# oss0430/SRFRD

Hardware: NVIDIA B200
Metric: training seqs/sec; full-catalogue top-10 users/sec (higher is better)
Workload: dtype bf16

## Files before the change

include/srfrd_b200.h:

```cpp
#ifndef SRFRD_B200_H
#define SRFRD_B200_H

#include <stddef.h>
#include <stdint.h>

#ifdef __cplusplus
extern "C" {
#endif

#define SRFRD_ABI_VERSION 9
#if defined(__GNUC__)
#define SRFRD_API __attribute__((visibility("default")))
#else
#define SRFRD_API
#endif

SRFRD_API const char* srfrd_last_error(void);
SRFRD_API int srfrd_abi_version(void);
SRFRD_API int srfrd_device_check(void);

SRFRD_API int srfrd_embed_ln_fwd(const float* item_table, int64_t n_rows, int D, const float* pos_table,
                       const float* aux_table, int64_t n_aux, int F, int mode, const int64_t* seq,
                       const int64_t* aux_ids, int64_t B, int L, float item_scale, const float* ln_w,
                       const float* ln_b, float eps, void* x0_bf16, float* x0_f32, void* q_bf16, float* stats,
                       int ldx, float drop_p, uint64_t drop_seed, uint32_t drop_stream, const float* drop_step,
// ... 138 lines not shown
  int* last_row;
  int64_t cap;
} srfrd_pack_t;
SRFRD_API int srfrd_pack_plan(const int64_t* seq, const int64_t* keep, int64_t B, int L, const srfrd_pack_t* pk, void* stream);
SRFRD_API int srfrd_set_row_limit(const int* rows_dev);
SRFRD_API int srfrd_embed_ln_fwd_packed(const float* item_table, int64_t n_rows, int D, const float* pos_table,
                              const float* aux_table, int64_t n_aux, int F, int mode, const int64_t* seq,
                              const int64_t* aux_ids, int64_t B, int L, float item_scale, const float* ln_w,
                              const float* ln_b, float eps, void* x0_bf16, void* q_bf16, float* stats, int ldx,
                              float drop_p, uint64_t drop_seed, uint32_t drop_stream, const float* drop_step,
                              const int* row_tok, const int* rows_dev, int64_t cap_rows, void* stream);
SRFRD_API int srfrd_layernorm_fwd_rows(const void* x_bf16, int ldx, const float* w, const float* b, float eps, float* y_f32,
                             int ldy, const int* row_index, int64_t n, int H, void* stream);
SRFRD_API int srfrd_attention_packed_supported(int L, int H, int heads);
SRFRD_API int srfrd_attention_packed_oproj_supported(int L, int H, int heads);
SRFRD_API int srfrd_attention_fwd_packed(const void* q, int ldq, const void* k, const void* v, int ldkv, void* o, int ldo,
                               const srfrd_pack_t* pk, int L, int H, int heads, float drop_p, uint64_t seed,
                               uint32_t stream_id, const float* drop_step, void* stream, const void* wo, int ldw,
                               const float* bo, const void* res, int ldres, const float* ln_w, const float* ln_b,
                               float ln_eps, float* ln_stats, void* r, int ldr, void* y, int ldy);
SRFRD_API int srfrd_attention_bwd_packed(const void* dout, int lddo, const void* q, int ldq, const void* k, const void* v,
                               int ldkv, void* dq, int lddq, void* dk, void* dv, int lddkv, const srfrd_pack_t* pk,
                               int L, int H, int heads, float drop_p, uint64_t seed, uint32_t stream_id,
                               const float* drop_step, void* stream, const void* dr, int lddr, const void* woT, int ldw);
SRFRD_API int srfrd_score_loss_fused_packed(const float* h, int ldh, const float* item_table, const float* fake_table,
                                  const int64_t* pos, const int64_t* neg, const int64_t* prs, const int64_t* nrs,
                                  const float* w_pos, const float* w_neg, const float* norm, int D, int F,
                                  float* loss_acc, float* dh, int lddh, float* d_item, float* d_fake,
                                  const int* row_tok, const int* rows_dev, int64_t cap_rows, void* stream);
SRFRD_API int srfrd_embed_bwd_packed(const void* dx0_bf16, int ldx, const int64_t* seq, const int64_t* aux_ids,
                           const int* row_tok, const int* rows_dev, int64_t cap_rows, int L, int D, int F, int mode,
                           float item_scale, float* d_item, float* d_aux, float* d_pos, void* stream);

typedef struct {
  const float* bias1; const float* bias2;
// ... 38 lines not shown
```

srfrd_b200/_lib.py:

```python
from __future__ import annotations

import ctypes as C
import os

_HERE = os.path.dirname(os.path.abspath(__file__))
LIB_PATH = os.environ.get("SRFRD_B200_LIB") or os.path.join(_HERE, "lib", "libsrfrd_b200.so")

vp, i32, i64, f32, u32, u64 = C.c_void_p, C.c_int, C.c_int64, C.c_float, C.c_uint32, C.c_uint64


class GemmEpilogue(C.Structure):
    _fields_ = [("bias", vp), ("residual", vp), ("gate", vp), ("row_ids", vp), ("out_bf16", vp), ("out_f32", vp),
                ("ldr", i32), ("ldg", i32), ("ldc", i32), ("relu", i32), ("drop_p", f32), ("drop_stream", u32),
                ("drop_seed", u64), ("drop_step", vp),
                ("ln_out_bf16", vp), ("ln_w", vp), ("ln_b", vp), ("ln_stats", vp), ("ld_ln", i32), ("ln_eps", f32)]


class CastDesc(C.Structure):
    _fields_ = [("src", vp), ("src_ld", i32), ("dst", vp), ("dst_ld", i32), ("dst_t", vp), ("dst_t_ld", i32),
                ("rows", i32), ("cols", i32), ("dst_is_f32", i32)]


class Mlp2Epilogue(C.Structure):
    _fields_ = [("bias1", vp), ("bias2", vp), ("gate", vp), ("ldg", i32), ("relu1", i32), ("drop1_p", f32), ("drop2_p", f32),
# ... 51 lines not shown
    "srfrd_merge_topk_packed": [vp, i64, i32, i32, vp, vp, vp],
    "srfrd_catalogue_rank": [vp, i64, i64, i32, vp, i64, i64, i64, i32, i32, i32, vp, i32, vp, vp, vp, vp],
    "srfrd_attention_live_items": [vp, i64, i32, i32, vp, vp, vp, vp],
    "srfrd_set_attention_live": [vp, vp, vp, vp],
    "srfrd_merge_topk": [vp, vp, i64, i32, i32, vp, vp, vp],
    "srfrd_unpack_rows": [C.POINTER(RepackPart), i32, C.POINTER(PackDesc), i64, i32, vp],
    "srfrd_pack_rows": [C.POINTER(RepackPart), i32, C.POINTER(PackDesc), i64, i32, vp],
    "srfrd_dp_adam_step": [vp, vp, vp, i32, i32, i64, vp, vp, f32, f32, f32, f32, vp, vp, vp, vp, vp, i32, vp, vp],
    "srfrd_pack_plan": [vp, vp, i64, i32, C.POINTER(PackDesc), vp],
    "srfrd_set_row_limit": [vp],
    "srfrd_embed_ln_fwd_packed": [vp, i64, i32, vp, vp, i64, i32, i32, vp, vp, i64, i32, f32, vp, vp, f32, vp, vp, vp, i32,
                                  f32, u64, u32, vp, vp, vp, i64, vp],
    "srfrd_layernorm_fwd_rows": [vp, i32, vp, vp, f32, vp, i32, vp, i64, i32, vp],
    "srfrd_attention_packed_supported": [i32, i32, i32],
    "srfrd_attention_packed_oproj_supported": [i32, i32, i32],
    "srfrd_attention_fwd_packed": [vp, i32, vp, vp, i32, vp, i32, C.POINTER(PackDesc), i32, i32, i32, f32, u64, u32, vp, vp,
                                   vp, i32, vp, vp, i32, vp, vp, f32, vp, vp, i32, vp, i32],
    "srfrd_attention_bwd_packed": [vp, i32, vp, i32, vp, vp, i32, vp, i32, vp, vp, i32, C.POINTER(PackDesc), i32, i32, i32,
                                   f32, u64, u32, vp, vp, vp, i32, vp, i32],
    "srfrd_score_loss_fused_packed": [vp, i32, vp, vp, vp, vp, vp, vp, vp, vp, vp, i32, i32, vp, vp, i32, vp, vp, vp, vp,
                                      i64, vp],
    "srfrd_embed_bwd_packed": [vp, i32, vp, vp, vp, vp, i64, i32, i32, i32, i32, f32, vp, vp, vp, vp],
    "srfrd_sample_candidates": [vp, vp, vp, vp, i64, i32, i32, u64, vp, vp],
    "srfrd_candidate_rank": [vp, i32, vp, i64, i32, vp, i64, i32, vp, i32, vp, vp, i32, vp, vp, vp],
    "srfrd_add_user_term": [vp, i32, i64, i32, vp, i32, vp, vp, i32, vp],
    "srfrd_sample_batch": [vp, vp, vp, vp, vp, i32, i32, i32, i32, i32, u64, vp, vp, vp, vp, vp, vp, vp, vp, vp, vp],
}

_lib = None
_device_ok = False
launch_count = 0

# ... 1 lines not shown
def load() -> C.CDLL:
    global _lib
    if _lib is not None:
        return _lib
    if not os.path.exists(LIB_PATH):
        raise RuntimeError(
            f"srfrd_b200: {LIB_PATH} is not built. Run `make -C srfrd_b200/csrc` (needs nvcc, sm_100a). "
            "There is no CPU fallback.")
    lib = C.CDLL(LIB_PATH)
    lib.srfrd_last_error.restype = C.c_char_p
    lib.srfrd_last_error.argtypes = []
    for name, argtypes in SIGNATURES.items():
        fn = getattr(lib, name)
        fn.argtypes = argtypes
        fn.restype = C.c_int
    if lib.srfrd_abi_version() != 9:
        raise RuntimeError("srfrd_b200: ABI version mismatch between _lib.py and the built library")
    _lib = lib
    return lib


def require_device() -> None:
    global _device_ok
    if _device_ok:
        return
    lib = load()
    if lib.srfrd_device_check() != 0:
        raise RuntimeError("srfrd_b200: " + lib.srfrd_last_error().decode())
    _device_ok = True


# ... 24 lines not shown
```

srfrd_b200/csrc/attention_tc.cu:

```cuda
#include <stdlib.h>

#include "common.cuh"
#include "srfrd_b200.h"

namespace srfrd {

int attn_fwd_simt(const void* q, int ldq, const void* k, const void* v, int ldkv, void* o, int ldo, int64_t B, int L,
                  int H, int heads, float drop_p, uint64_t seed, uint32_t stream_id, const float* drop_step, void* stream);
int attn_bwd_simt(const void* dout, int lddo, const void* q, int ldq, const void* k, const void* v, int ldkv, void* dq,
                  int lddq, void* dk, void* dv, int lddkv, int64_t B, int L, int H, int heads, float drop_p,
                  uint64_t seed, uint32_t stream_id, const float* drop_step, void* stream);

bool attn_long_supported(int64_t B, int L, int H, int heads, int ldq, int ldkv);
int attn_long_fwd(const void* q, int ldq, const void* k, const void* v, int ldkv, void* o, int ldo, float* stats, int64_t B,
                  int L, int H, int heads, float drop_p, uint64_t seed, uint32_t stream_id, const float* drop_step,
                  void* stream);
int attn_long_bwd(const void* dout, int lddo, const void* q, int ldq, const void* k, const void* v, int ldkv, const void* o,
                  int ldo, float* stats, void* dq, int lddq, void* dk, void* dv, int lddkv, int64_t B, int L, int H, int heads,
                  float drop_p, uint64_t seed, uint32_t stream_id, const float* drop_step, void* stream);

static constexpr int TILE = 128;
static constexpr int OPB = TILE * 64 * 2;
static constexpr int ATC_THREADS = 192;

struct AttnTc {
  int64_t T;
  int L, hd, heads, spt, n_tiles, kblocks;
  int tma_o;
  int debug;
  float scale, scale_log2e;
  bf16* o; int ldo;
  bf16 *dq, *dk, *dv; int lddq, lddkv;
  uint64_t drop_seed; uint32_t drop_thresh, drop_stream; float drop_scale; const float* drop_step;
  const int* pk_rows;
  const int4* pk_info;
  const int* pk_tile_row0;
  const float *op_bias, *ln_w, *ln_b; float* ln_stats; float ln_eps;
  bf16 *op_r, *op_y; int ldr, ldy;
};

__device__ __forceinline__ uint32_t sw128(int r, int c) {
  return (uint32_t)(r * 128 + ((((c >> 3) ^ (r & 7)) << 4) | ((c & 7) << 1)));
}

struct RowInfo {
  int r; int64_t t; bool owned; int jlo, jhi, l; int64_t bh;
  float pm;
  int jbase;
};
__device__ __forceinline__ RowInfo row_info_pk(const AttnTc& p, int row0, int M, int h, int quarter, int lane) {
  RowInfo ri;
  ri.r = quarter * 32 + lane;
  ri.t = (int64_t)row0 + ri.r;
// ... 108 lines not shown
  return y;
}

__device__ __forceinline__ void store_staged_rows(bf16* dst, int ld, int64_t row0, int col0, const uint8_t* blocks, int hd,
                                                  int n_own, int tid256) {
  const int cpr = hd >> 3;
  for (int i = tid256; i < n_own * cpr; i += 256) {
    const int r = i / cpr, ch = i - r * cpr;
    const uint4 v = *reinterpret_cast<const uint4*>(blocks + (ch >> 3) * OPB + sw128(r, (ch & 7) * 8));
    *reinterpret_cast<uint4*>(dst + (row0 + r) * ld + col0 + ch * 8) = v;
  }
}

static constexpr int AF_THREADS = 320;

__device__ __forceinline__ void out_proj_epilogue(const AttnTc& p, uint8_t* Qs, uint8_t* Vs, float* xsum, float* xsq,
                                               const float* sop, uint32_t tacc, uint64_t* proj_full, uint64_t* w_full,
                                               uint32_t ph, int r, int part, int quarter, int row0, int n_own) {
  mbar_wait2(proj_full, ph, w_full, ph);
  tc_fence_after();
  float ln_sum = 0.f, ln_sq = 0.f;
#pragma unroll 1
  for (int c = part * 32; c < p.hd; c += 64) {
    uint32_t raw[32];
    tmem_ld32(tacc + c, raw);
    uint8_t* blk = Vs + (c >> 6) * OPB;
    uint4 ax[4];
#pragma unroll
    for (int j = 0; j < 4; ++j)
      if (c + 8 * j < p.hd) ax[j] = *reinterpret_cast<const uint4*>(blk + sw128(r, (c & 63) + 8 * j));
// ... 20 lines not shown
  for (int c = part * 32; c < p.hd; c += 64) {
#pragma unroll
    for (int j = 0; j < 4; ++j) {
      if (c + 8 * j >= p.hd) break;
      const uint32_t off = (c >> 6) * OPB + sw128(r, (c & 63) + 8 * j);
      *reinterpret_cast<uint4*>(Qs + off) =
          lnf_apply8(*reinterpret_cast<const uint4*>(Vs + off), rstd, nb, sop + TILE + c + 8 * j, sop + 2 * TILE + c + 8 * j);
    }
  }
  if (part == 0 && r < n_own && p.ln_stats) *reinterpret_cast<float2*>(p.ln_stats + 2 * (size_t)(row0 + r)) = make_float2(mean, rstd);
  named_bar_sync_a(9, 256);
  store_staged_rows(p.op_r, p.ldr, row0, 0, Vs, p.hd, n_own, threadIdx.x);
  store_staged_rows(p.op_y, p.ldy, row0, 0, Qs, p.hd, n_own, threadIdx.x);
}

template <bool DROP, bool PK, bool OP>
__global__ void __launch_bounds__(AF_THREADS, 2)
attn_fwd_tc_kernel(const __grid_constant__ CUtensorMap tmQ, const __grid_constant__ CUtensorMap tmK,
                   const __grid_constant__ CUtensorMap tmV, const __grid_constant__ CUtensorMap tmO,
                   const __grid_constant__ CUtensorMap tmW, const __grid_constant__ CUtensorMap tmR, AttnTc p) {
  extern __shared__ uint8_t smem_raw[];
  uint8_t* smem = reinterpret_cast<uint8_t*>((reinterpret_cast<uintptr_t>(smem_raw) + 1023) & ~uintptr_t(1023));
  const int opbytes = p.kblocks * OPB;
  uint8_t* Qs = smem;
  uint8_t* Ks = Qs + opbytes;
  uint8_t* Vs = Ks + max(p.kblocks, 2) * OPB;
  float* smax = reinterpret_cast<float*>(Vs + opbytes);
  float* ssum = smax + 2 * TILE;
  uint64_t* bars = reinterpret_cast<uint64_t*>(ssum + 2 * TILE);
  uint64_t *qk_full = bars, *v_full = bars + 1, *s_full = bars + 2, *p_full = bars + 3, *o_full = bars + 4,
           *kv_free = bars + 5, *q_free = bars + 6;
  uint64_t *w_full = bars + 7, *o_staged = bars + 8, *proj_full = bars + 9;
  uint32_t* tmem_slot = reinterpret_cast<uint32_t*>(bars + 10);
  float* sop = reinterpret_cast<float*>(bars + 16);
  const int warp = threadIdx.x >> 5, lane = threadIdx.x & 31;

  if (warp == 8 && lane == 0) {
    tma_prefetch_desc(&tmQ); tma_prefetch_desc(&tmK); tma_prefetch_desc(&tmV); tma_prefetch_desc(&tmO);
    if (OP) { tma_prefetch_desc(&tmW); tma_prefetch_desc(&tmR); }
    mbar_init(qk_full, 1); mbar_init(v_full, 1); mbar_init(s_full, 1); mbar_init(p_full, 8); mbar_init(o_full, 1);
    mbar_init(kv_free, 1); mbar_init(q_free, 1);
    mbar_init(w_full, 1); mbar_init(o_staged, 1); mbar_init(proj_full, 1);
    fence_barrier_init();
  }
  if (warp == 9) { tmem_alloc(tmem_slot, 256); tmem_relinquish(); }
  tc_fence_before();
  __syncthreads();
  tc_fence_after();
  const uint32_t tmem_base = *tmem_slot;
  const uint32_t tS = tmem_base, tO = tmem_base + 128;
  pdl_prologue_done();
  if (DROP) p.drop_seed = mix_seed(p.drop_seed, p.drop_step);
  const int pk_M = PK ? __ldg(p.pk_rows) : 0;
  const int n_items = (PK ? __ldg(p.pk_rows + 2) : p.n_tiles) * p.heads;

  if (warp == 8) {
    uint32_t ph = 0;
    for (int it = blockIdx.x; it < n_items; it += gridDim.x, ph ^= 1) {
      const int tile = it / p.heads, h = it % p.heads;
      const int row0 = PK ? __ldg(p.pk_tile_row0 + tile) : tile * p.spt * p.L, col0 = h * p.hd;
      mbar_wait(q_free, ph ^ 1);
      if (!OP) mbar_wait(kv_free, ph ^ 1);
      AT_STAMP(0, it / gridDim.x);
      if (elect_one()) {
        mbar_expect_tx(qk_full, 2 * opbytes);
        for (int kb = 0; kb < p.kblocks; ++kb) {
          tma_load_2d(Qs + kb * OPB, &tmQ, qk_full, col0 + kb * 64, row0, SRFRD_EVICT_FIRST);
          tma_load_2d(Ks + kb * OPB, &tmK, qk_full, col0 + kb * 64, row0, SRFRD_EVICT_FIRST);
        }
        mbar_expect_tx(v_full, opbytes);
        for (int kb = 0; kb < p.kblocks; ++kb)
          tma_load_2d(Vs + kb * OPB, &tmV, v_full, col0 + kb * 64, row0, SRFRD_EVICT_FIRST);
      }
      __syncwarp();
      if (OP) {
        mbar_wait(kv_free, ph);
        if (elect_one()) {
          mbar_expect_tx(w_full, p.kblocks * (p.hd * 128 + OPB));
          for (int kb = 0; kb < p.kblocks; ++kb) {
            tma_load_2d(Ks + kb * OPB, &tmW, w_full, kb * 64, 0, SRFRD_EVICT_LAST);
            tma_load_2d(Vs + kb * OPB, &tmR, w_full, kb * 64, row0, SRFRD_EVICT_FIRST);
          }
        }
        __syncwarp();
      }
    }
  } else if (warp == 9) {
    const uint32_t idS = umma_idesc_bf16(TILE, TILE, 0, 0);
    const uint32_t idO = umma_idesc_bf16(TILE, p.hd, 0, 1);
    const uint32_t idW = umma_idesc_bf16(TILE, p.hd, 0, 0);
    const uint64_t dQ = umma_smem_desc(smem_u32(Qs), 0, 1024), dK = umma_smem_desc(smem_u32(Ks), 0, 1024);
    const uint64_t dP = umma_smem_desc(smem_u32(Ks), 0, 1024), dV = umma_smem_desc(smem_u32(Vs), OPB, 1024);
    uint32_t ph = 0;
    for (int it = blockIdx.x; it < n_items; it += gridDim.x, ph ^= 1) {
      mbar_wait(qk_full, ph);
      tc_fence_after();
      AT_STAMP(1, it / gridDim.x);
      if (elect_one()) {
        for (int kb = 0; kb < p.kblocks; ++kb) {
          const int ksteps = min(4, (p.hd - kb * 64) / 16);
          for (int k = 0; k < ksteps; ++k)
            umma_bf16(tS, dQ + (uint64_t)(kb * (OPB >> 4) + 2 * k), dK + (uint64_t)(kb * (OPB >> 4) + 2 * k), idS, (kb | k) != 0);
        }
        umma_commit(s_full);
      }
      __syncwarp();
      AT_STAMP(2, it / gridDim.x);
      mbar_wait(p_full, ph);
      mbar_wait(v_full, ph);
      tc_fence_after();
      AT_STAMP(3, it / gridDim.x);
      if (elect_one()) {
#pragma unroll
        for (int ks = 0; ks < 8; ++ks)
          umma_bf16(tO, dP + (uint64_t)((ks >> 2) * (OPB >> 4) + (ks & 3) * 2), dV + (uint64_t)(ks * 128), idO, ks != 0);
        umma_commit(kv_free);
        umma_commit(o_full);
      }
      __syncwarp();
      AT_STAMP(4, it / gridDim.x);
      if (OP) {
        mbar_wait2(o_staged, ph, w_full, ph);
        tc_fence_after();
        if (elect_one()) {
// ... 6 lines not shown
        }
        __syncwarp();
      }
    }
  } else {
    const int quarter = warp & 3, part = warp >> 2;
    const uint32_t lane_off = (uint32_t)(quarter * 32) << 16;
    const int r_first = quarter * 32;
    const int c_lo = PK ? (max(0, r_first - p.L) >> 5) : min(((r_first / p.L) * p.L) >> 5, quarter), c_hi = quarter;
    if (OP)
      for (int i = threadIdx.x; i < TILE; i += 256) {
        sop[i] = (p.op_bias && i < p.hd) ? __ldg(p.op_bias + i) : 0.f;
        sop[TILE + i] = i < p.hd ? __ldg(p.ln_w + i) : 0.f;
        sop[2 * TILE + i] = i < p.hd ? __ldg(p.ln_b + i) : 0.f;
      }
    uint32_t ph = 0;
    for (int it = blockIdx.x; it < n_items; it += gridDim.x, ph ^= 1) {
      const int tile = it / p.heads, h = it % p.heads;
      const int pk_row0 = PK ? __ldg(p.pk_tile_row0 + tile) : 0;
      RowInfo ri = PK ? row_info_pk(p, pk_row0, pk_M, h, quarter, lane) : row_info(p, tile, h, quarter, lane);
      if (!ri.owned) { ri.jlo = 1 << 20; ri.jhi = ri.jlo; }
      const unsigned span = (unsigned)(ri.jhi - ri.jlo);
      mbar_wait(s_full, ph);
      tc_fence_after();
      if (warp == 0) AT_STAMP(5, it / gridDim.x);
      const int c0 = c_lo + part, c1 = c_lo + part + 2;
      const int lo0 = (c0 <= c_hi) ? ri.jlo - c0 * 32 : (1 << 20);
      const int lo1 = (c1 <= c_hi) ? ri.jlo - c1 * 32 : (1 << 20);
      uint32_t raw0[32], raw1[32];
      tmem_ld32(tS + lane_off + min(c0, c_hi) * 32, raw0);
      tmem_ld32(tS + lane_off + min(c1, c_hi) * 32, raw1);
      tmem_ld_wait();
      float m = -INFINITY;
#pragma unroll
// ... 558 lines not shown
                          tmDO, tmDQ, tmDK, tmDV, tmDV, p));
  SRFRD_LAUNCH_CHECK();
  return 0;
}

static int packed_supported(int L, int H, int heads, int ldq, int ldkv) {
  if (!tc_supported(L, H, heads, ldq, ldkv)) return 0;
  const int hd = H / heads;
  return (L + 1 <= TILE) && (heads == 1 || hd % 64 == 0);
}

extern "C" int srfrd_attention_packed_supported(int L, int H, int heads) {
  return packed_supported(L, H, heads, 8, 8) && !getenv("SRFRD_ATTN_SIMT");
}

static size_t fwd_smem(int kblocks, bool op) {
  return (size_t)(2 * kblocks + (kblocks > 2 ? kblocks : 2)) * OPB + 4 * TILE * sizeof(float) + 1024 + 256 +
         (op ? 3 * TILE * sizeof(float) : 0);
}
static size_t bwd_smem(int kblocks, int hd, bool op) {
  return op ? (size_t)(4 * kblocks + 4) * OPB + 4096 + (size_t)kblocks * hd * 128 + 1024
            : (size_t)(4 * kblocks + 4) * OPB + 6 * TILE * sizeof(float) + 1024 + 256;
}
static constexpr size_t FWD_SMEM_MAX = 113 * 1024;
static constexpr size_t BWD_SMEM_MAX = 227 * 1024;

static int oproj_supported(int L, int H, int heads) {
  if (!packed_supported(L, H, heads, 8, 8) || heads != 1 || H > 128) return 0;
  const int kblocks = (H + 63) / 64;
  return (fwd_smem(kblocks, true) <= FWD_SMEM_MAX ? 1 : 0) | (bwd_smem(kblocks, H, true) <= BWD_SMEM_MAX ? 2 : 0);
}

extern "C" int srfrd_attention_packed_oproj_supported(int L, int H, int heads) {
  return getenv("SRFRD_ATTN_SIMT") ? 0 : oproj_supported(L, H, heads);
}

extern "C" int srfrd_attention_fwd_packed(const void* q, int ldq, const void* k, const void* v, int ldkv, void* o, int ldo,
                                          const srfrd_pack_t* pk, int L, int H, int heads, float drop_p, uint64_t seed,
                                          uint32_t stream_id, const float* drop_step, void* stream, const void* wo, int ldw,
                                          const float* bo, const void* res, int ldres, const float* ln_w, const float* ln_b,
                                          float ln_eps, float* ln_stats, void* r, int ldr, void* y, int ldy) {
  SRFRD_REQUIRE(q && k && v && o && pk && pk->rows && pk->row_info && pk->tile_row0, "attention_fwd_packed: null pointer");
  SRFRD_REQUIRE(packed_supported(L, H, heads, ldq, ldkv) && ldo % 8 == 0 && ((uintptr_t)o & 15) == 0,
                "attention_fwd_packed: unsupported shape (L=%d H=%d heads=%d)", L, H, heads);
  const bool op = wo != nullptr;
  if (op) {
    SRFRD_REQUIRE(oproj_supported(L, H, heads) & 1, "attention_fwd_packed: no fused out-projection for H=%d heads=%d", H, heads);
    SRFRD_REQUIRE(res && ln_w && ln_b && r && y, "attention_fwd_packed: fused out-projection needs residual, LayerNorm, r and y");
    SRFRD_REQUIRE(ldw % 8 == 0 && ldw >= H && ldres % 8 == 0 && ldr % 8 == 0 && ldy % 8 == 0 &&
                      (((uintptr_t)res | (uintptr_t)r | (uintptr_t)y | (uintptr_t)wo) & 15) == 0,
                  "attention_fwd_packed: bad out-projection operands");
  }
  AttnTc p = {};
  if (int rc = fill(p, 1, L, H, heads, drop_p, seed, stream_id, drop_step)) return rc;
  p.T = pk->cap;
  p.o = (bf16*)o; p.ldo = ldo; p.tma_o = 1;
  p.pk_rows = pk->rows; p.pk_info = (const int4*)pk->row_info; p.pk_tile_row0 = pk->tile_row0;
  CUtensorMap tmQ, tmK, tmV, tmW, tmR;
  if (int rc = make_tmap_bf16_2d(&tmQ, q, p.T, H, ldq, TILE, 64)) return rc;
  if (int rc = make_tmap_bf16_2d(&tmK, k, p.T, H, ldkv, TILE, 64)) return rc;
  if (int rc = make_tmap_bf16_2d(&tmV, v, p.T, H, ldkv, TILE, 64)) return rc;
  tmW = tmQ; tmR = tmQ;
  if (op) {
    if (int rc = make_tmap_bf16_2d(&tmW, wo, H, H, ldw, H, 64)) return rc;
    if (int rc = make_tmap_bf16_2d(&tmR, res, p.T, H, ldres, TILE, 64)) return rc;
    p.op_bias = bo; p.ln_w = ln_w; p.ln_b = ln_b; p.ln_stats = ln_stats; p.ln_eps = ln_eps;
    p.op_r = (bf16*)r; p.op_y = (bf16*)y; p.ldr = ldr; p.ldy = ldy;
  }
  const size_t smem = fwd_smem(p.kblocks, op);
  static bool attr = false;
  if (!attr) {
    SRFRD_CUDA(cudaFuncSetAttribute(attn_fwd_tc_kernel<false, true, false>, cudaFuncAttributeMaxDynamicSharedMemorySize, FWD_SMEM_MAX));
    SRFRD_CUDA(cudaFuncSetAttribute(attn_fwd_tc_kernel<true, true, false>, cudaFuncAttributeMaxDynamicSharedMemorySize, FWD_SMEM_MAX));
    SRFRD_CUDA(cudaFuncSetAttribute(attn_fwd_tc_kernel<false, true, true>, cudaFuncAttributeMaxDynamicSharedMemorySize, FWD_SMEM_MAX));
    SRFRD_CUDA(cudaFuncSetAttribute(attn_fwd_tc_kernel<true, true, true>, cudaFuncAttributeMaxDynamicSharedMemorySize, FWD_SMEM_MAX));
    attr = true;
  }
  int64_t grid = (pk->cap / 64 + 1) * heads;
  if (grid > 2 * num_sms()) grid = 2 * num_sms();
  auto kern = p.drop_thresh ? (op ? attn_fwd_tc_kernel<true, true, true> : attn_fwd_tc_kernel<true, true, false>)
                            : (op ? attn_fwd_tc_kernel<false, true, true> : attn_fwd_tc_kernel<false, true, false>);
  SRFRD_CUDA(launch_pdl(kern, dim3((unsigned)grid), dim3(AF_THREADS), smem, (cudaStream_t)stream, tmQ, tmK, tmV, tmQ, tmW, tmR, p));
  SRFRD_LAUNCH_CHECK();
  return 0;
}

extern "C" int srfrd_attention_bwd_packed(const void* dout, int lddo, const void* q, int ldq, const void* k, const void* v,
                                          int ldkv, void* dq, int lddq, void* dk, void* dv, int lddkv, const srfrd_pack_t* pk,
                                          int L, int H, int heads, float drop_p, uint64_t seed, uint32_t stream_id,
                                          const float* drop_step, void* stream, const void* dr, int lddr, const void* woT,
                                          int ldw) {
  const bool op = dr != nullptr;
  SRFRD_REQUIRE((op ? (woT != nullptr) : (dout != nullptr)) && q && k && v && dq && dk && dv && pk && pk->rows &&
                    pk->row_info && pk->tile_row0,
                "attention_bwd_packed: null pointer");
  SRFRD_REQUIRE(packed_supported(L, H, heads, ldq, ldkv) && (op || lddo % 8 == 0) && lddq % 8 == 0 && lddkv % 8 == 0 &&
                    (((uintptr_t)dq | (uintptr_t)dk | (uintptr_t)dv) & 15) == 0,
// ... 38 lines not shown
```

srfrd_b200/engine.py:

```python
from __future__ import annotations

import math
import os
from contextlib import contextmanager, nullcontext
from dataclasses import dataclass
from typing import Dict, List, Optional, Tuple

import torch

from . import ops

bf16 = torch.bfloat16
LN_EPS = 1e-8

KINDS = ("SRFR", "SRFRN", "SRFU_B", "SRFU_F", "SRFU_R", "SASRec")


@dataclass
class ModelSpec:
    kind: str
    item_number: int
    max_len: int
    D: int
    F: int = 0
# ... 491 lines not shown
            need = {"SRFU_B": 3, "SRFU_F": L + 1, "SRFU_R": 11}[s.kind]
            if s.n_labels < need and int(aux_ids.max()) >= s.n_labels:
                raise IndexError(f"index out of range in self: {s.kind} user label {int(aux_ids.max())} needs "
                                 f"number_of_labels >= {need}, got {s.n_labels}")
        aux_table = P.view(s.aux_key) if s.aux_key else None
        plan.build(seq, None if keep is None else keep.contiguous())
        hyb = self._hybrid_ws(B * L) if self.packed_mode(B, L) == "hybrid" else None
        live = None
        if hyb is not None and os.environ.get("SRFRD_LIVE_TILES", "1") != "0":
            live = self._live_tiles(B, L)
            live.build(plan)
        x = [ws[f"x{i}"][:T] for i in range(nb + 1)]
        row_ids = plan.row_ids
        fuse_ln = Hp <= 128 and os.environ.get("SRFRD_FUSE_LN", "1") != "0"
        fuse_oproj = self._fuse_oproj(hyb, L, fuse_ln) & 1
        with ops.row_limit(plan.rows):
            ops.embed_ln_fwd_packed(P.view(s.item_key), P.view(s.pos_key), aux_table, s.mode, seq, aux_ids, s.item_scale,
                                    P.view("attention_layernorms.0.weight"), P.view("attention_layernorms.0.bias"), LN_EPS,
                                    x[0], ws["Q0"][:T], ws["st1_0"][:T], plan,
                                    drop_p=p_drop if s.kind == "SASRec" else 0.0, drop_seed=seed, drop_stream=1, drop_step=step)
            for i in range(nb):
                Q, q, kv, o, r, y, h1 = (ws[f"{n}{i}"][:T] for n in ("Q", "q", "kv", "o", "r", "y", "h1"))
                with self._branch():
                    ops.gemm_tn(x[i], self.sh[f"wkv{i}"], out_bf16=kv, bias=self.bias("bkv", i))
                if i > 0 and not fuse_ln:
                    ops.layernorm_fwd(x[i], P.view(f"attention_layernorms.{i}.weight"), P.view(f"attention_layernorms.{i}.bias"),
                                      LN_EPS, y_bf16=Q, stats=ws[f"st1_{i}"][:T], H=H)
                ops.gemm_tn(Q, self.sh[f"wq{i}"], out_bf16=q, bias=self.bias("bq", i))
                self._join()
                if fuse_oproj:
                    ops.attention_fwd_packed(q, kv[:, :Hp], kv[:, Hp:], o, plan, L, H, s.num_heads, p_drop, seed, 10 + 4 * i, step,
                                             wo=self.sh[f"wo{i}"], bias=self.bias("bo", i), residual=Q, r=r, y=y,
                                             ln_w=P.view(f"forward_layernorms.{i}.weight"),
                                             ln_b=P.view(f"forward_layernorms.{i}.bias"), ln_eps=LN_EPS,
                                             ln_stats=ws[f"st2_{i}"][:T])
                elif hyb is None:
                    ops.attention_fwd_packed(q, kv[:, :Hp], kv[:, Hp:], o, plan, L, H, s.num_heads, p_drop, seed, 10 + 4 * i, step)
                else:
                    qd, kvd, od = hyb[f"qd{i}"][:B * L], hyb[f"kvd{i}"][:B * L], hyb[f"od{i}"][:B * L]
                    ops.unpack_rows([(q, qd, Hp, 0), (kv, kvd, 2 * Hp, 0)], plan)
                    with (live.active() if live is not None else nullcontext()):
                        ops.attention_fwd(qd, kvd[:, :Hp], kvd[:, Hp:], od, B, L, H, s.num_heads, p_drop, seed, 10 + 4 * i, step,
                                          stats=ws.get(f"ast{i}"))
                    ops.pack_rows([(od, o, Hp, 0)], plan)
                if fuse_oproj:
                    pass
                elif fuse_ln:
                    ops.gemm_tn(o, self.sh[f"wo{i}"], out_bf16=r, bias=self.bias("bo", i), residual=Q, ln_out=y,
                                ln_w=P.view(f"forward_layernorms.{i}.weight"), ln_b=P.view(f"forward_layernorms.{i}.bias"),
                                ln_eps=LN_EPS, ln_stats=ws[f"st2_{i}"][:T])
# ... 140 lines not shown
```

srfrd_b200/ops.py:

```python
from __future__ import annotations

import ctypes as C
from typing import Optional

import torch

from . import _lib
from contextlib import contextmanager

from ._lib import CastDesc, GemmEpilogue, Mlp2Epilogue, PackDesc, RepackPart, call

bf16 = torch.bfloat16


def _p(t: Optional[torch.Tensor]):
    return None if t is None else t.data_ptr()


def _stream():
    return torch.cuda.current_stream().cuda_stream


def _chk(t: torch.Tensor, dtype, name: str):
    if not t.is_cuda:
# ... 346 lines not shown
         0 if aux_table is None else aux_table.shape[0], F, mode, _p(seq), _p(aux_ids), B, L, float(item_scale), _p(ln_w),
         _p(ln_b), float(eps), _p(x0_bf16), _p(q_bf16), _p(stats), x0_bf16.stride(0), float(drop_p), int(drop_seed),
         int(drop_stream), _p(drop_step), _p(plan.row_tok), _p(plan.rows), plan.cap, _stream())


def layernorm_fwd_rows(x, w, b, eps, y_f32, row_index, n, H):
    _lib.require_device()
    call("srfrd_layernorm_fwd_rows", _p(x), x.stride(0), _p(w), _p(b), float(eps), _p(y_f32), y_f32.stride(0), _p(row_index),
         n, H, _stream())


def attention_packed_oproj_supported(L: int, H: int, heads: int) -> int:
    return int(_lib.load().srfrd_attention_packed_oproj_supported(int(L), int(H), int(heads)))


def attention_fwd_packed(q, k, v, o, plan: PackedPlan, L, H, heads, drop_p=0.0, seed=0, stream_id=0, drop_step=None,
                         wo=None, bias=None, residual=None, r=None, y=None, ln_w=None, ln_b=None, ln_eps=0.0, ln_stats=None):
    _lib.require_device()
    st = lambda t: 0 if t is None else t.stride(0)
    call("srfrd_attention_fwd_packed", _p(q), q.stride(0), _p(k), _p(v), k.stride(0), _p(o), o.stride(0), C.byref(plan.desc),
         L, H, heads, float(drop_p), int(seed), int(stream_id), _p(drop_step), _stream(), _p(wo), st(wo), _p(bias),
         _p(residual), st(residual), _p(ln_w), _p(ln_b), float(ln_eps), _p(ln_stats), _p(r), st(r), _p(y), st(y))


def attention_bwd_packed(dout, q, k, v, dq, dk, dv, plan: PackedPlan, L, H, heads, drop_p=0.0, seed=0, stream_id=0,
                         drop_step=None, dr=None, woT=None):
    st = lambda t: 0 if t is None else t.stride(0)
    call("srfrd_attention_bwd_packed", _p(dout), st(dout), _p(q), q.stride(0), _p(k), _p(v), k.stride(0), _p(dq),
         dq.stride(0), _p(dk), _p(dv), dk.stride(0), C.byref(plan.desc), L, H, heads, float(drop_p), int(seed),
         int(stream_id), _p(drop_step), _stream(), _p(dr), st(dr), _p(woT), st(woT))


def score_loss_fused_packed(h, item_table, fake_table, pos, neg, prs, nrs, w_pos, w_neg, norm, loss_acc, dh, d_item, d_fake,
                            plan: PackedPlan):
    D = item_table.shape[1]
    F = 0 if fake_table is None else fake_table.shape[1]
    call("srfrd_score_loss_fused_packed", _p(h), h.stride(0), _p(item_table), _p(fake_table), _p(pos), _p(neg), _p(prs),
# ... 49 lines not shown
```

Before: 9.857 million.

## Fuse Q and KV input projections into packed attention forward kernel

Adds an in-projection variant of the packed tensor-core attention forward kernel. It loads the raw Q input, the KV input and the Wq/Wkv weights by TMA, computes the Q, K and V projections with UMMA into TMEM, adds the biases and stages the results in shared memory. It also writes them to global memory, because the backward pass still needs them. The engine uses this path, and skips the separate wkv and wq GEMM launches plus the branch/join, whenever the fused out-projection is already active and the shape fits in TMEM and shared memory. The aim is fewer launches and less global round-tripping of q/kv, at the cost of more shared memory, serialized weight loads inside the kernel, and possibly repeated projection work per head item.

After: 10.03 million, median of 6. 1.02x the previous value.

```diff
diff --git a/include/srfrd_b200.h b/include/srfrd_b200.h
--- a/include/srfrd_b200.h
+++ b/include/srfrd_b200.h
@@ -8,7 +8,7 @@
 extern "C" {
 #endif
 
-#define SRFRD_ABI_VERSION 9
+#define SRFRD_ABI_VERSION 10
 #if defined(__GNUC__)
 #define SRFRD_API __attribute__((visibility("default")))
 #else
@@ -177,11 +177,14 @@
                              int ldy, const int* row_index, int64_t n, int H, void* stream);
 SRFRD_API int srfrd_attention_packed_supported(int L, int H, int heads);
 SRFRD_API int srfrd_attention_packed_oproj_supported(int L, int H, int heads);
+SRFRD_API int srfrd_attention_packed_inproj_supported(int L, int H, int heads);
 SRFRD_API int srfrd_attention_fwd_packed(const void* q, int ldq, const void* k, const void* v, int ldkv, void* o, int ldo,
                                const srfrd_pack_t* pk, int L, int H, int heads, float drop_p, uint64_t seed,
                                uint32_t stream_id, const float* drop_step, void* stream, const void* wo, int ldw,
                                const float* bo, const void* res, int ldres, const float* ln_w, const float* ln_b,
-                               float ln_eps, float* ln_stats, void* r, int ldr, void* y, int ldy);
+                               float ln_eps, float* ln_stats, void* r, int ldr, void* y, int ldy, const void* q_in,
+                               int ldq_in, const void* kv_in, int ldkv_in, const void* wq, int ldwq, const void* wkv,
+                               int ldwkv, const float* bq, const float* bkv);
 SRFRD_API int srfrd_attention_bwd_packed(const void* dout, int lddo, const void* q, int ldq, const void* k, const void* v,
                                int ldkv, void* dq, int lddq, void* dk, void* dv, int lddkv, const srfrd_pack_t* pk,
                                int L, int H, int heads, float drop_p, uint64_t seed, uint32_t stream_id,
diff --git a/srfrd_b200/_lib.py b/srfrd_b200/_lib.py
--- a/srfrd_b200/_lib.py
+++ b/srfrd_b200/_lib.py
@@ -89,8 +89,10 @@
     "srfrd_layernorm_fwd_rows": [vp, i32, vp, vp, f32, vp, i32, vp, i64, i32, vp],
     "srfrd_attention_packed_supported": [i32, i32, i32],
     "srfrd_attention_packed_oproj_supported": [i32, i32, i32],
+    "srfrd_attention_packed_inproj_supported": [i32, i32, i32],
     "srfrd_attention_fwd_packed": [vp, i32, vp, vp, i32, vp, i32, C.POINTER(PackDesc), i32, i32, i32, f32, u64, u32, vp, vp,
-                                   vp, i32, vp, vp, i32, vp, vp, f32, vp, vp, i32, vp, i32],
+                                   vp, i32, vp, vp, i32, vp, vp, f32, vp, vp, i32, vp, i32, vp, i32, vp, i32, vp, i32, vp, i32,
+                                   vp, vp],
     "srfrd_attention_bwd_packed": [vp, i32, vp, i32, vp, vp, i32, vp, i32, vp, vp, i32, C.POINTER(PackDesc), i32, i32, i32,
                                    f32, u64, u32, vp, vp, vp, i32, vp, i32],
     "srfrd_score_loss_fused_packed": [vp, i32, vp, vp, vp, vp, vp, vp, vp, vp, vp, i32, i32, vp, vp, i32, vp, vp, vp, vp,
@@ -122,7 +124,7 @@
         fn = getattr(lib, name)
         fn.argtypes = argtypes
         fn.restype = C.c_int
-    if lib.srfrd_abi_version() != 9:
+    if lib.srfrd_abi_version() != 10:
         raise RuntimeError("srfrd_b200: ABI version mismatch between _lib.py and the built library")
     _lib = lib
     return lib
diff --git a/srfrd_b200/csrc/attention_tc.cu b/srfrd_b200/csrc/attention_tc.cu
--- a/srfrd_b200/csrc/attention_tc.cu
+++ b/srfrd_b200/csrc/attention_tc.cu
@@ -37,6 +37,8 @@
   const int* pk_tile_row0;
   const float *op_bias, *ln_w, *ln_b; float* ln_stats; float ln_eps;
   bf16 *op_r, *op_y; int ldr, ldy;
+  const float *ip_bq, *ip_bkv;
+  bf16 *ip_q, *ip_k, *ip_v; int ip_ldq, ip_ldkv;
 };
 
 __device__ __forceinline__ uint32_t sw128(int r, int c) {
@@ -175,6 +177,50 @@
 
 static constexpr int AF_THREADS = 320;
 
+__device__ __forceinline__ void umma_in_proj(uint32_t tacc, uint64_t da, uint64_t db, uint32_t idesc, int hd) {
+  for (int kb = 0; kb * 64 < hd; ++kb) {
+    const int ksteps = min(4, (hd - kb * 64) / 16);
+    for (int k = 0; k < ksteps; ++k)
+      umma_bf16(tacc, da + (uint64_t)(kb * (OPB >> 4) + 2 * k), db + (uint64_t)(kb * (OPB >> 4) + 2 * k), idesc, (kb | k) != 0);
+  }
+}
+
+__device__ __forceinline__ void in_proj_epilogue(const AttnTc& p, uint8_t* Qs, uint8_t* Ks, uint8_t* Vs, const float* sip,
+                                              uint32_t tacc, uint64_t* qkv_full, uint64_t* qkv_staged, uint32_t ph, int r,
+                                              int part, int warp, int lane, int row0, int n_own) {
+  mbar_wait(qkv_full, ph);
+  tc_fence_after();
+  const bool own = r < n_own;
+#pragma unroll 1
+  for (int m = 0; m < 3; ++m) {
+    uint8_t* dst = m == 0 ? Qs : (m == 1 ? Ks : Vs);
+    bf16* gdst = m == 0 ? p.ip_q + (size_t)(row0 + r) * p.ip_ldq
+                        : (m == 1 ? p.ip_k : p.ip_v) + (size_t)(row0 + r) * p.ip_ldkv;
+    const float* bias = sip + m * TILE;
+#pragma unroll 1
+    for (int c = part * 32; c < p.hd; c += 64) {
+      uint32_t ro[32];
+      tmem_ld32(tacc + m * p.hd + c, ro);
+      tmem_ld_wait();
+      uint8_t* blk = dst + (c >> 6) * OPB;
+#pragma unroll
+      for (int u = 0; u < 4; ++u) {
+        if (c + 8 * u >= p.hd) break;
+        float v[8];
+#pragma unroll
+        for (int j = 0; j < 8; ++j) v[j] = __uint_as_float(ro[8 * u + j]) + bias[c + 8 * u + j];
+        const uint4 pk = make_uint4(pack_bf16x2(v[0], v[1]), pack_bf16x2(v[2], v[3]), pack_bf16x2(v[4], v[5]), pack_bf16x2(v[6], v[7]));
+        *reinterpret_cast<uint4*>(blk + sw128(r, (c & 63) + 8 * u)) = pk;
+        if (own) *reinterpret_cast<uint4*>(gdst + c + 8 * u) = pk;
+      }
+    }
+  }
+  tc_fence_before();
+  fence_proxy_async();
+  named_bar_sync_a(9, 256);
+  if (warp == 0 && lane == 0) mbar_arrive(qkv_staged);
+}
+
 __device__ __forceinline__ void out_proj_epilogue(const AttnTc& p, uint8_t* Qs, uint8_t* Vs, float* xsum, float* xsq,
                                                const float* sop, uint32_t tacc, uint64_t* proj_full, uint64_t* w_full,
                                                uint32_t ph, int r, int part, int quarter, int row0, int n_own) {
@@ -225,11 +271,12 @@
   store_staged_rows(p.op_y, p.ldy, row0, 0, Qs, p.hd, n_own, threadIdx.x);
 }
 
-template <bool DROP, bool PK, bool OP>
+template <bool DROP, bool PK, bool OP, bool IP = false>
 __global__ void __launch_bounds__(AF_THREADS, 2)
 attn_fwd_tc_kernel(const __grid_constant__ CUtensorMap tmQ, const __grid_constant__ CUtensorMap tmK,
                    const __grid_constant__ CUtensorMap tmV, const __grid_constant__ CUtensorMap tmO,
                    const __grid_constant__ CUtensorMap tmW, const __grid_constant__ CUtensorMap tmR, AttnTc p) {
+  static_assert(!IP || (PK && OP), "the fused in-projection runs on the packed, out-projection form only");
   extern __shared__ uint8_t smem_raw[];
   uint8_t* smem = reinterpret_cast<uint8_t*>((reinterpret_cast<uintptr_t>(smem_raw) + 1023) & ~uintptr_t(1023));
   const int opbytes = p.kblocks * OPB;
@@ -244,6 +291,9 @@
   uint64_t *w_full = bars + 7, *o_staged = bars + 8, *proj_full = bars + 9;
   uint32_t* tmem_slot = reinterpret_cast<uint32_t*>(bars + 10);
   float* sop = reinterpret_cast<float*>(bars + 16);
+  float* sip = sop + 3 * TILE;
+  uint64_t* ipbars = reinterpret_cast<uint64_t*>(sip + 3 * TILE);
+  uint64_t *q_done = ipbars, *ipw_full = ipbars + 1, *qkv_full = ipbars + 2, *qkv_staged = ipbars + 3;
   const int warp = threadIdx.x >> 5, lane = threadIdx.x & 31;
 
   if (warp == 8 && lane == 0) {
@@ -252,6 +302,7 @@
     mbar_init(qk_full, 1); mbar_init(v_full, 1); mbar_init(s_full, 1); mbar_init(p_full, 8); mbar_init(o_full, 1);
     mbar_init(kv_free, 1); mbar_init(q_free, 1);
     mbar_init(w_full, 1); mbar_init(o_staged, 1); mbar_init(proj_full, 1);
+    if (IP) { mbar_init(q_done, 1); mbar_init(ipw_full, 1); mbar_init(qkv_full, 1); mbar_init(qkv_staged, 1); }
     fence_barrier_init();
   }
   if (warp == 9) { tmem_alloc(tmem_slot, 256); tmem_relinquish(); }
@@ -273,7 +324,26 @@
       mbar_wait(q_free, ph ^ 1);
       if (!OP) mbar_wait(kv_free, ph ^ 1);
       AT_STAMP(0, it / gridDim.x);
-      if (elect_one()) {
+      if (IP) {
+        const int wbytes = p.hd * 128;
+        if (elect_one()) {
+          mbar_expect_tx(qk_full, 2 * opbytes + p.kblocks * wbytes);
+          for (int kb = 0; kb < p.kblocks; ++kb) {
+            tma_load_2d(Qs + kb * OPB, &tmQ, qk_full, kb * 64, row0, SRFRD_EVICT_FIRST);
+            tma_load_2d(Ks + kb * OPB, &tmK, qk_full, kb * 64, row0, SRFRD_EVICT_FIRST);
+            tma_load_2d(Vs + kb * OPB, &tmO, qk_full, kb * 64, 0, SRFRD_EVICT_LAST);
+          }
+        }
+        __syncwarp();
+        mbar_wait(q_done, ph);
+        if (elect_one()) {
+          mbar_expect_tx(ipw_full, 2 * p.kblocks * wbytes);
+          for (int kb = 0; kb < p.kblocks; ++kb) {
+            tma_load_2d(Vs + kb * OPB, &tmV, ipw_full, kb * 64, 0, SRFRD_EVICT_LAST);
+            tma_load_2d(Qs + kb * OPB, &tmV, ipw_full, kb * 64, p.hd, SRFRD_EVICT_LAST);
+          }
+        }
+      } else if (elect_one()) {
         mbar_expect_tx(qk_full, 2 * opbytes);
         for (int kb = 0; kb < p.kblocks; ++kb) {
           tma_load_2d(Qs + kb * OPB, &tmQ, qk_full, col0 + kb * 64, row0, SRFRD_EVICT_FIRST);
@@ -304,7 +374,27 @@
     const uint64_t dP = umma_smem_desc(smem_u32(Ks), 0, 1024), dV = umma_smem_desc(smem_u32(Vs), OPB, 1024);
     uint32_t ph = 0;
     for (int it = blockIdx.x; it < n_items; it += gridDim.x, ph ^= 1) {
-      mbar_wait(qk_full, ph);
+      if (IP) {
+        const uint64_t dVk = umma_smem_desc(smem_u32(Vs), 0, 1024);
+        mbar_wait(qk_full, ph);
+        tc_fence_after();
+        if (elect_one()) {
+          umma_in_proj(tmem_base, dQ, dVk, idW, p.hd);
+          umma_commit(q_done);
+        }
+        __syncwarp();
+        mbar_wait(ipw_full, ph);
+        tc_fence_after();
+        if (elect_one()) {
+          umma_in_proj(tmem_base + p.hd, dK, dVk, idW, p.hd);
+          umma_in_proj(tmem_base + 2 * p.hd, dK, dQ, idW, p.hd);
+          umma_commit(qkv_full);
+        }
+        __syncwarp();
+        mbar_wait(qkv_staged, ph);
+      } else {
+        mbar_wait(qk_full, ph);
+      }
       tc_fence_after();
       AT_STAMP(1, it / gridDim.x);
       if (elect_one()) {
@@ -318,7 +408,7 @@
       __syncwarp();
       AT_STAMP(2, it / gridDim.x);
       mbar_wait(p_full, ph);
-      mbar_wait(v_full, ph);
+      if (!IP) mbar_wait(v_full, ph);
       tc_fence_after();
       AT_STAMP(3, it / gridDim.x);
       if (elect_one()) {
@@ -355,10 +445,21 @@
         sop[TILE + i] = i < p.hd ? __ldg(p.ln_w + i) : 0.f;
         sop[2 * TILE + i] = i < p.hd ? __ldg(p.ln_b + i) : 0.f;
       }
+    if (IP) {
+      for (int i = threadIdx.x; i < TILE; i += 256) {
+        sip[i] = (p.ip_bq && i < p.hd) ? __ldg(p.ip_bq + i) : 0.f;
+        sip[TILE + i] = (p.ip_bkv && i < p.hd) ? __ldg(p.ip_bkv + i) : 0.f;
+        sip[2 * TILE + i] = (p.ip_bkv && i < p.hd) ? __ldg(p.ip_bkv + p.hd + i) : 0.f;
+      }
+      named_bar_sync_a(9, 256);
+    }
     uint32_t ph = 0;
     for (int it = blockIdx.x; it < n_items; it += gridDim.x, ph ^= 1) {
       const int tile = it / p.heads, h = it % p.heads;
       const int pk_row0 = PK ? __ldg(p.pk_tile_row0 + tile) : 0;
+      if (IP)
+        in_proj_epilogue(p, Qs, Ks, Vs, sip, tmem_base + lane_off, qkv_full, qkv_staged, ph, quarter * 32 + lane, part, warp,
+                         lane, pk_row0, __ldg(p.pk_tile_row0 + tile + 1) - pk_row0);
       RowInfo ri = PK ? row_info_pk(p, pk_row0, pk_M, h, quarter, lane) : row_info(p, tile, h, quarter, lane);
       if (!ri.owned) { ri.jlo = 1 << 20; ri.jhi = ri.jlo; }
       const unsigned span = (unsigned)(ri.jhi - ri.jlo);
@@ -947,9 +1048,9 @@
   return packed_supported(L, H, heads, 8, 8) && !getenv("SRFRD_ATTN_SIMT");
 }
 
-static size_t fwd_smem(int kblocks, bool op) {
+static size_t fwd_smem(int kblocks, bool op, bool ip = false) {
   return (size_t)(2 * kblocks + (kblocks > 2 ? kblocks : 2)) * OPB + 4 * TILE * sizeof(float) + 1024 + 256 +
-         (op ? 3 * TILE * sizeof(float) : 0);
+         (op ? 3 * TILE * sizeof(float) : 0) + (ip ? 3 * TILE * sizeof(float) + 64 : 0);
 }
 static size_t bwd_smem(int kblocks, int hd, bool op) {
   return op ? (size_t)(4 * kblocks + 4) * OPB + 4096 + (size_t)kblocks * hd * 128 + 1024
@@ -968,15 +1069,34 @@
   return getenv("SRFRD_ATTN_SIMT") ? 0 : oproj_supported(L, H, heads);
 }
 
+static bool inproj_supported(int L, int H, int heads) {
+  return (oproj_supported(L, H, heads) & 1) && 3 * H <= 256 && fwd_smem((H + 63) / 64, true, true) <= FWD_SMEM_MAX;
+}
+
+extern "C" int srfrd_attention_packed_inproj_supported(int L, int H, int heads) {
+  return !getenv("SRFRD_ATTN_SIMT") && inproj_supported(L, H, heads);
+}
+
 extern "C" int srfrd_attention_fwd_packed(const void* q, int ldq, const void* k, const void* v, int ldkv, void* o, int ldo,
                                           const srfrd_pack_t* pk, int L, int H, int heads, float drop_p, uint64_t seed,
                                           uint32_t stream_id, const float* drop_step, void* stream, const void* wo, int ldw,
                                           const float* bo, const void* res, int ldres, const float* ln_w, const float* ln_b,
-                                          float ln_eps, float* ln_stats, void* r, int ldr, void* y, int ldy) {
+                                          float ln_eps, float* ln_stats, void* r, int ldr, void* y, int ldy,
+                                          const void* q_in, int ldq_in, const void* kv_in, int ldkv_in, const void* wq,
+                                          int ldwq, const void* wkv, int ldwkv, const float* bq, const float* bkv) {
   SRFRD_REQUIRE(q && k && v && o && pk && pk->rows && pk->row_info && pk->tile_row0, "attention_fwd_packed: null pointer");
   SRFRD_REQUIRE(packed_supported(L, H, heads, ldq, ldkv) && ldo % 8 == 0 && ((uintptr_t)o & 15) == 0,
                 "attention_fwd_packed: unsupported shape (L=%d H=%d heads=%d)", L, H, heads);
-  const bool op = wo != nullptr;
+  const bool op = wo != nullptr, ip = wq != nullptr;
+  if (ip) {
+    SRFRD_REQUIRE(op && inproj_supported(L, H, heads), "attention_fwd_packed: no fused in-projection for H=%d heads=%d%s", H,
+                  heads, op ? "" : " without the fused out-projection");
+    SRFRD_REQUIRE(q_in && kv_in && wkv, "attention_fwd_packed: fused in-projection needs q_in, kv_in and wkv");
+    SRFRD_REQUIRE(ldq_in % 8 == 0 && ldkv_in % 8 == 0 && ldwq % 8 == 0 && ldwq >= H && ldwkv % 8 == 0 && ldwkv >= H &&
+                      (((uintptr_t)q_in | (uintptr_t)kv_in | (uintptr_t)wq | (uintptr_t)wkv | (uintptr_t)q | (uintptr_t)k |
+                        (uintptr_t)v) & 15) == 0,
+                  "attention_fwd_packed: bad in-projection operands");
+  }
   if (op) {
     SRFRD_REQUIRE(oproj_supported(L, H, heads) & 1, "attention_fwd_packed: no fused out-projection for H=%d heads=%d", H, heads);
     SRFRD_REQUIRE(res && ln_w && ln_b && r && y, "attention_fwd_packed: fused out-projection needs residual, LayerNorm, r and y");
@@ -989,10 +1109,20 @@
   p.T = pk->cap;
   p.o = (bf16*)o; p.ldo = ldo; p.tma_o = 1;
   p.pk_rows = pk->rows; p.pk_info = (const int4*)pk->row_info; p.pk_tile_row0 = pk->tile_row0;
-  CUtensorMap tmQ, tmK, tmV, tmW, tmR;
-  if (int rc = make_tmap_bf16_2d(&tmQ, q, p.T, H, ldq, TILE, 64)) return rc;
-  if (int rc = make_tmap_bf16_2d(&tmK, k, p.T, H, ldkv, TILE, 64)) return rc;
-  if (int rc = make_tmap_bf16_2d(&tmV, v, p.T, H, ldkv, TILE, 64)) return rc;
+  CUtensorMap tmQ, tmK, tmV, tmW, tmR, tmWq;
+  if (ip) {
+    if (int rc = make_tmap_bf16_2d(&tmQ, q_in, p.T, H, ldq_in, TILE, 64)) return rc;
+    if (int rc = make_tmap_bf16_2d(&tmK, kv_in, p.T, H, ldkv_in, TILE, 64)) return rc;
+    if (int rc = make_tmap_bf16_2d(&tmV, wkv, 2 * H, H, ldwkv, H, 64)) return rc;
+    if (int rc = make_tmap_bf16_2d(&tmWq, wq, H, H, ldwq, H, 64)) return rc;
+    p.ip_bq = bq; p.ip_bkv = bkv;
+    p.ip_q = (bf16*)q; p.ip_k = (bf16*)k; p.ip_v = (bf16*)v; p.ip_ldq = ldq; p.ip_ldkv = ldkv;
+  } else {
+    if (int rc = make_tmap_bf16_2d(&tmQ, q, p.T, H, ldq, TILE, 64)) return rc;
+    if (int rc = make_tmap_bf16_2d(&tmK, k, p.T, H, ldkv, TILE, 64)) return rc;
+    if (int rc = make_tmap_bf16_2d(&tmV, v, p.T, H, ldkv, TILE, 64)) return rc;
+    tmWq = tmQ;
+  }
   tmW = tmQ; tmR = tmQ;
   if (op) {
     if (int rc = make_tmap_bf16_2d(&tmW, wo, H, H, ldw, H, 64)) return rc;
@@ -1000,20 +1130,24 @@
     p.op_bias = bo; p.ln_w = ln_w; p.ln_b = ln_b; p.ln_stats = ln_stats; p.ln_eps = ln_eps;
     p.op_r = (bf16*)r; p.op_y = (bf16*)y; p.ldr = ldr; p.ldy = ldy;
   }
-  const size_t smem = fwd_smem(p.kblocks, op);
+  const size_t smem = fwd_smem(p.kblocks, op, ip);
   static bool attr = false;
   if (!attr) {
     SRFRD_CUDA(cudaFuncSetAttribute(attn_fwd_tc_kernel<false, true, false>, cudaFuncAttributeMaxDynamicSharedMemorySize, FWD_SMEM_MAX));
     SRFRD_CUDA(cudaFuncSetAttribute(attn_fwd_tc_kernel<true, true, false>, cudaFuncAttributeMaxDynamicSharedMemorySize, FWD_SMEM_MAX));
     SRFRD_CUDA(cudaFuncSetAttribute(attn_fwd_tc_kernel<false, true, true>, cudaFuncAttributeMaxDynamicSharedMemorySize, FWD_SMEM_MAX));
     SRFRD_CUDA(cudaFuncSetAttribute(attn_fwd_tc_kernel<true, true, true>, cudaFuncAttributeMaxDynamicSharedMemorySize, FWD_SMEM_MAX));
+    SRFRD_CUDA(cudaFuncSetAttribute(attn_fwd_tc_kernel<false, true, true, true>, cudaFuncAttributeMaxDynamicSharedMemorySize, FWD_SMEM_MAX));
+    SRFRD_CUDA(cudaFuncSetAttribute(attn_fwd_tc_kernel<true, true, true, true>, cudaFuncAttributeMaxDynamicSharedMemorySize, FWD_SMEM_MAX));
     attr = true;
   }
   int64_t grid = (pk->cap / 64 + 1) * heads;
   if (grid > 2 * num_sms()) grid = 2 * num_sms();
-  auto kern = p.drop_thresh ? (op ? attn_fwd_tc_kernel<true, true, true> : attn_fwd_tc_kernel<true, true, false>)
-                            : (op ? attn_fwd_tc_kernel<false, true, true> : attn_fwd_tc_kernel<false, true, false>);
-  SRFRD_CUDA(launch_pdl(kern, dim3((unsigned)grid), dim3(AF_THREADS), smem, (cudaStream_t)stream, tmQ, tmK, tmV, tmQ, tmW, tmR, p));
+  auto kern = p.drop_thresh ? (ip ? attn_fwd_tc_kernel<true, true, true, true>
+                                  : op ? attn_fwd_tc_kernel<true, true, true> : attn_fwd_tc_kernel<true, true, false>)
+                            : (ip ? attn_fwd_tc_kernel<false, true, true, true>
+                                  : op ? attn_fwd_tc_kernel<false, true, true> : attn_fwd_tc_kernel<false, true, false>);
+  SRFRD_CUDA(launch_pdl(kern, dim3((unsigned)grid), dim3(AF_THREADS), smem, (cudaStream_t)stream, tmQ, tmK, tmV, tmWq, tmW, tmR, p));
   SRFRD_LAUNCH_CHECK();
   return 0;
 }
diff --git a/srfrd_b200/engine.py b/srfrd_b200/engine.py
--- a/srfrd_b200/engine.py
+++ b/srfrd_b200/engine.py
@@ -529,6 +529,7 @@
         row_ids = plan.row_ids
         fuse_ln = Hp <= 128 and os.environ.get("SRFRD_FUSE_LN", "1") != "0"
         fuse_oproj = self._fuse_oproj(hyb, L, fuse_ln) & 1
+        fuse_inproj = fuse_oproj and ops.attention_packed_inproj_supported(L, H, s.num_heads)
         with ops.row_limit(plan.rows):
             ops.embed_ln_fwd_packed(P.view(s.item_key), P.view(s.pos_key), aux_table, s.mode, seq, aux_ids, s.item_scale,
                                     P.view("attention_layernorms.0.weight"), P.view("attention_layernorms.0.bias"), LN_EPS,
@@ -536,19 +537,22 @@
                                     drop_p=p_drop if s.kind == "SASRec" else 0.0, drop_seed=seed, drop_stream=1, drop_step=step)
             for i in range(nb):
                 Q, q, kv, o, r, y, h1 = (ws[f"{n}{i}"][:T] for n in ("Q", "q", "kv", "o", "r", "y", "h1"))
-                with self._branch():
-                    ops.gemm_tn(x[i], self.sh[f"wkv{i}"], out_bf16=kv, bias=self.bias("bkv", i))
-                if i > 0 and not fuse_ln:
-                    ops.layernorm_fwd(x[i], P.view(f"attention_layernorms.{i}.weight"), P.view(f"attention_layernorms.{i}.bias"),
-                                      LN_EPS, y_bf16=Q, stats=ws[f"st1_{i}"][:T], H=H)
-                ops.gemm_tn(Q, self.sh[f"wq{i}"], out_bf16=q, bias=self.bias("bq", i))
-                self._join()
+                if not fuse_inproj:
+                    with self._branch():
+                        ops.gemm_tn(x[i], self.sh[f"wkv{i}"], out_bf16=kv, bias=self.bias("bkv", i))
+                    if i > 0 and not fuse_ln:
+                        ops.layernorm_fwd(x[i], P.view(f"attention_layernorms.{i}.weight"),
+                                          P.view(f"attention_layernorms.{i}.bias"), LN_EPS, y_bf16=Q, stats=ws[f"st1_{i}"][:T], H=H)
+                    ops.gemm_tn(Q, self.sh[f"wq{i}"], out_bf16=q, bias=self.bias("bq", i))
+                    self._join()
+                inproj = dict(q_in=Q, kv_in=x[i], wq=self.sh[f"wq{i}"], wkv=self.sh[f"wkv{i}"], bq=self.bias("bq", i),
+                              bkv=self.bias("bkv", i)) if fuse_inproj else {}
                 if fuse_oproj:
                     ops.attention_fwd_packed(q, kv[:, :Hp], kv[:, Hp:], o, plan, L, H, s.num_heads, p_drop, seed, 10 + 4 * i, step,
                                              wo=self.sh[f"wo{i}"], bias=self.bias("bo", i), residual=Q, r=r, y=y,
                                              ln_w=P.view(f"forward_layernorms.{i}.weight"),
                                              ln_b=P.view(f"forward_layernorms.{i}.bias"), ln_eps=LN_EPS,
-                                             ln_stats=ws[f"st2_{i}"][:T])
+                                             ln_stats=ws[f"st2_{i}"][:T], **inproj)
                 elif hyb is None:
                     ops.attention_fwd_packed(q, kv[:, :Hp], kv[:, Hp:], o, plan, L, H, s.num_heads, p_drop, seed, 10 + 4 * i, step)
                 else:
diff --git a/srfrd_b200/ops.py b/srfrd_b200/ops.py
--- a/srfrd_b200/ops.py
+++ b/srfrd_b200/ops.py
@@ -384,13 +384,19 @@
     return int(_lib.load().srfrd_attention_packed_oproj_supported(int(L), int(H), int(heads)))
 
 
+def attention_packed_inproj_supported(L: int, H: int, heads: int) -> bool:
+    return bool(_lib.load().srfrd_attention_packed_inproj_supported(int(L), int(H), int(heads)))
+
+
 def attention_fwd_packed(q, k, v, o, plan: PackedPlan, L, H, heads, drop_p=0.0, seed=0, stream_id=0, drop_step=None,
-                         wo=None, bias=None, residual=None, r=None, y=None, ln_w=None, ln_b=None, ln_eps=0.0, ln_stats=None):
+                         wo=None, bias=None, residual=None, r=None, y=None, ln_w=None, ln_b=None, ln_eps=0.0, ln_stats=None,
+                         q_in=None, kv_in=None, wq=None, wkv=None, bq=None, bkv=None):
     _lib.require_device()
     st = lambda t: 0 if t is None else t.stride(0)
     call("srfrd_attention_fwd_packed", _p(q), q.stride(0), _p(k), _p(v), k.stride(0), _p(o), o.stride(0), C.byref(plan.desc),
          L, H, heads, float(drop_p), int(seed), int(stream_id), _p(drop_step), _stream(), _p(wo), st(wo), _p(bias),
-         _p(residual), st(residual), _p(ln_w), _p(ln_b), float(ln_eps), _p(ln_stats), _p(r), st(r), _p(y), st(y))
+         _p(residual), st(residual), _p(ln_w), _p(ln_b), float(ln_eps), _p(ln_stats), _p(r), st(r), _p(y), st(y),
+         _p(q_in), st(q_in), _p(kv_in), st(kv_in), _p(wq), st(wq), _p(wkv), st(wkv), _p(bq), _p(bkv))
 
 
 def attention_bwd_packed(dout, q, k, v, dq, dk, dv, plan: PackedPlan, L, H, heads, drop_p=0.0, seed=0, stream_id=0,
```
